# facebookresearch/EgoT2

Hardware: NVIDIA B200
Metric: translator fwd+bwd clips/sec (higher is better)
Workload: dtype bf16

## Files before the change

### egot2_b200/csrc/gemm_sm100.cu

```cuda
#include <stdio.h>
#include <stdlib.h>

#define EGOT2_FILE_ID 4
#include "ops.h"
#include "sm100.cuh"

namespace egot2 {

using namespace sm100;

namespace {

constexpr int BM = 128;
constexpr int BK = 64;
#ifndef EGOT2_GEMM_EPG
#define EGOT2_GEMM_EPG 1
#endif
constexpr int EPG = EGOT2_GEMM_EPG;
constexpr int NTHREADS = 64 + 128 * EPG;

struct EpiArgs {
  int M, N;
  void* C; int ldc; int c_rpg, c_gstride;
  const float* bias; int relu;
  const void* mask; int ldm; float mask_scale;
  float p_drop; uint64_t drop_key; int drop_bit_mode;
  const void* residual; int ldr;
  int accumulate; int atomic;
  long long split_stride;
  int tma_store;
  int k_grouped, kg, kdblocks;
  const float* ln_g; const float* ln_b; float ln_eps;
  void* ln_out; float* ln_stat; const float* ln_table; int ln_table_rows; int ln_row0;
  float ln_p_drop; uint64_t ln_drop_key;
  int trans_c;
  int tma_red;
  int trace_slot;
};

#ifdef EGOT2_GEMM_TRACE
__device__ long long g_gtrace[512][16];
#define GTR(k) do { if (blockIdx.x == 0 && blockIdx.z == 0 && e.trace_slot >= 0) g_gtrace[e.trace_slot][k] = clock64(); } while (0)
#else
#define GTR(k) do { } while (0)
#endif

__device__ __forceinline__ long long remap(int r, int rpg, int gstride) {
  return rpg > 0 ? (long long)(r / rpg) * gstride + (r % rpg) : (long long)r;
}


__device__ __forceinline__ void red_add_v4(float* p, float a, float b, float c, float d) {
  asm volatile("red.global.add.v4.f32 [%0], {%1, %2, %3, %4};" ::"l"(p), "f"(a), "f"(b), "f"(c), "f"(d) : "memory");
}

__device__ __forceinline__ bool aligned16(const void* p) { return (reinterpret_cast<uintptr_t>(p) & 15) == 0; }

__device__ __forceinline__ void load32(const float* p, float (&o)[32]) {
#pragma unroll
  for (int j = 0; j < 32; j += 4) {
    const float4 t = *reinterpret_cast<const float4*>(p + j);
    o[j] = t.x; o[j + 1] = t.y; o[j + 2] = t.z; o[j + 3] = t.w;
  }
}
__device__ __forceinline__ void load32(const bf16* p, float (&o)[32]) {
#pragma unroll
  for (int j = 0; j < 32; j += 8) {
    const uint4 t = *reinterpret_cast<const uint4*>(p + j);
    const uint32_t w[4] = {t.x, t.y, t.z, t.w};
#pragma unroll
    for (int k = 0; k < 4; ++k) {
      o[j + 2 * k] = __uint_as_float(w[k] << 16);
      o[j + 2 * k + 1] = __uint_as_float(w[k] & 0xffff0000u);
    }
  }
}
__device__ __forceinline__ void store32(float* p, const float (&v)[32]) {
#pragma unroll
  for (int j = 0; j < 32; j += 4) *reinterpret_cast<float4*>(p + j) = make_float4(v[j], v[j + 1], v[j + 2], v[j + 3]);
}
__device__ __forceinline__ void store32(bf16* p, const float (&v)[32]) {
#pragma unroll
  for (int j = 0; j < 32; j += 8) {
    uint4 o;
    __nv_bfloat162 p0 = __floats2bfloat162_rn(v[j], v[j + 1]), p1 = __floats2bfloat162_rn(v[j + 2], v[j + 3]);
    __nv_bfloat162 p2 = __floats2bfloat162_rn(v[j + 4], v[j + 5]), p3 = __floats2bfloat162_rn(v[j + 6], v[j + 7]);
    o.x = *reinterpret_cast<uint32_t*>(&p0); o.y = *reinterpret_cast<uint32_t*>(&p1);
    o.z = *reinterpret_cast<uint32_t*>(&p2); o.w = *reinterpret_cast<uint32_t*>(&p3);
    *reinterpret_cast<uint4*>(p + j) = o;
  }
}

template <int BN, typename TO> struct TileCfg {
  static constexpr uint32_t OUT_BYTES = (BN <= 128 && sizeof(TO) == 2) ? 128 * BN * 2 : 0;
  static constexpr int STAGES = BN == 128 ? (OUT_BYTES ? 2 : 3) : (BN == 64 ? (OUT_BYTES ? 3 : 4) : 4);
  static constexpr int MIN_CTAS = BN == 256 ? 1 : 2;
};
__device__ __forceinline__ void sts128(uint32_t dst, uint32_t a, uint32_t b, uint32_t c, uint32_t d) {
  asm volatile("st.shared.v4.b32 [%0], {%1, %2, %3, %4};" ::"r"(dst), "r"(a), "r"(b), "r"(c), "r"(d) : "memory");
}

__device__ __forceinline__ void named_bar_sync(int id, int n) { asm volatile("bar.sync %0, %1;" ::"r"(id), "r"(n) : "memory"); }

template <int BN, bool A_MN, bool B_MN, typename TO>
__global__ void __launch_bounds__(NTHREADS, TileCfg<BN, TO>::MIN_CTAS)
gemm_sm100_kernel(const __grid_constant__ CUtensorMap tma_a, const __grid_constant__ CUtensorMap tma_b,
                  const __grid_constant__ CUtensorMap tma_c, const EpiArgs e, const int k_blocks_total, const int k_blocks_per_split, const int tiles_n, const int num_tiles) {
  constexpr uint32_t A_BYTES = BM * BK * 2;
  constexpr uint32_t B_BYTES = BN * BK * 2;
  constexpr int STAGES = TileCfg<BN, TO>::STAGES;
  extern __shared__ uint8_t smem_raw[];
  const uint32_t smem_base = (smem_u32(smem_raw) + 1023u) & ~1023u;
  const uint32_t sA = smem_base;
  const uint32_t sB = sA + STAGES * A_BYTES;
  const uint32_t sOut = sB + STAGES * B_BYTES;
  const uint32_t bars = sOut + TileCfg<BN, TO>::OUT_BYTES;
  const uint32_t full0 = bars, empty0 = bars + 8 * STAGES, tmem_full = bars + 16 * STAGES, tmem_empty = tmem_full + 16;
  const uint32_t tmem_slot = tmem_empty + 16;
  const uint32_t bias_off = (tmem_slot + 8 + 15u) & ~15u;
  uint32_t* tmem_slot_ptr = reinterpret_cast<uint32_t*>(smem_raw + (tmem_slot - smem_u32(smem_raw)));

  const int warp = threadIdx.x >> 5, lane = threadIdx.x & 31;
  const int kb_begin = blockIdx.z * k_blocks_per_split;
  const int kb_end = min(k_blocks_total, kb_begin + k_blocks_per_split);
  const int nkb = kb_end - kb_begin;

  pdl_launch_dependents();
  if (threadIdx.x == 0) GTR(0);
  if (warp == 0 && lane == 0) {
    tma_prefetch_desc(&tma_a);
    tma_prefetch_desc(&tma_b);
    if (e.tma_store || e.tma_red) tma_prefetch_desc(&tma_c);
    for (int s = 0; s < STAGES; ++s) { mbar_init(full0 + 8 * s, 1); mbar_init(empty0 + 8 * s, 1); }
    for (int s = 0; s < 2; ++s) { mbar_init(tmem_full + 8 * s, 1); mbar_init(tmem_empty + 8 * s, 4 * EPG); }
    fence_barrier_init();
  }
  const bool one_tile = gridDim.z > 1;
  if (warp == 1) { if (one_tile) tmem_alloc<BN>(tmem_slot); else tmem_alloc<2 * BN>(tmem_slot); }
  if (threadIdx.x == 0) GTR(1);
  pdl_wait();
  if (threadIdx.x == 0) GTR(2);
  EGOT2_TL(EGOT2_FILE_ID);
  const unsigned long long egot2_ep = epoch_xor();
  float* sbias = reinterpret_cast<float*>(smem_raw + (bias_off - smem_u32(smem_raw)));
  tc_fence_before();
  __syncthreads();
  tc_fence_after();
  const uint32_t tmem_base = *tmem_slot_ptr;
  if (threadIdx.x == 0) GTR(3);

  if (warp == 0) {
    if (lane == 0) {
      int it = 0;
      for (int tile = blockIdx.x; tile < num_tiles; tile += gridDim.x) {
        const int m0 = (tile / tiles_n) * BM, n0 = (tile % tiles_n) * BN;
        for (int i = 0; i < nkb; ++i, ++it) {
          const int s = it % STAGES;
          const uint32_t ph = (it / STAGES) & 1;
          mbar_wait(empty0 + 8 * s, ph ^ 1);
          mbar_expect_tx(full0 + 8 * s, A_BYTES + B_BYTES);
          const int kb = kb_begin + i;
          const int k = kb * BK;
          if (A_MN && B_MN && e.k_grouped) {
            const int grp = (kb / e.kdblocks) * e.kg, d0 = (kb % e.kdblocks) * 64;
#pragma unroll
            for (int j = 0; j < BM / 64; ++j) tma_load_3d(sA + s * A_BYTES + j * 8192, &tma_a, full0 + 8 * s, m0 + 64 * j, d0, grp);
#pragma unroll
            for (int j = 0; j < BN / 64; ++j) tma_load_3d(sB + s * B_BYTES + j * 8192, &tma_b, full0 + 8 * s, n0 + 64 * j, d0, grp);
            continue;
          }
          if (!A_MN) {
            tma_load_2d(sA + s * A_BYTES, &tma_a, full0 + 8 * s, k, m0);
          } else {
#pragma unroll
            for (int j = 0; j < BM / 64; ++j) tma_load_2d(sA + s * A_BYTES + j * 8192, &tma_a, full0 + 8 * s, m0 + 64 * j, k);
          }
          if (!B_MN) {
            tma_load_2d(sB + s * B_BYTES, &tma_b, full0 + 8 * s, k, n0);
          } else {
#pragma unroll
            for (int j = 0; j < BN / 64; ++j) tma_load_2d(sB + s * B_BYTES + j * 8192, &tma_b, full0 + 8 * s, n0 + 64 * j, k);
          }
          if (tile == (int)blockIdx.x && (i == 0 || i == nkb - 1)) GTR(i == 0 ? 4 : 5);
        }
      }
    }
  } else if (warp == 1) {
    if (lane == 0) {
      constexpr uint32_t idesc = make_idesc_bf16(BM, BN, A_MN, B_MN);
      int it = 0, lt = 0;
      for (int tile = blockIdx.x; tile < num_tiles; tile += gridDim.x, ++lt) {
        const int buf = lt & 1;
        mbar_wait(tmem_empty + 8 * buf, ((lt >> 1) & 1) ^ 1);
        tc_fence_after();
        for (int i = 0; i < nkb; ++i, ++it) {
          const int s = it % STAGES;
          const uint32_t ph = (it / STAGES) & 1;
          mbar_wait(full0 + 8 * s, ph);
          if (lt == 0 && (i == 0 || i == nkb - 1)) GTR(i == 0 ? 6 : 7);
          tc_fence_after();
#pragma unroll
          for (int kk = 0; kk < BK / 16; ++kk) {
            const uint64_t ad = A_MN ? make_smem_desc_sw128(sA + s * A_BYTES + kk * 2048, 8192, 1024)
                                     : make_smem_desc_sw128(sA + s * A_BYTES + kk * 32, 16, 1024);
            const uint64_t bd = B_MN ? make_smem_desc_sw128(sB + s * B_BYTES + kk * 2048, 8192, 1024)
                                     : make_smem_desc_sw128(sB + s * B_BYTES + kk * 32, 16, 1024);
            umma_bf16(tmem_base + buf * BN, ad, bd, idesc, (i > 0 || kk > 0) ? 1u : 0u);
          }
          umma_commit(empty0 + 8 * s);
        }
        umma_commit(tmem_full + 8 * buf);
      }
    }
  } else {
    const int q = warp & 3;
    const int c_lo = ((warp - 2) >> 2) * (BN / EPG), c_hi = c_lo + BN / EPG;
    const float inv_keep = e.p_drop > 0.f ? 1.f / (1.f - e.p_drop) : 1.f;
    const bool first_split = blockIdx.z == 0;
    const float* bias = first_split ? e.bias : nullptr;
    const bool tma_red = sizeof(TO) == 4 && e.tma_red && gridDim.z > 1 && nkb > 0;
    int lt = 0;
    for (int tile = blockIdx.x; tile < num_tiles; tile += gridDim.x, ++lt) {
      const int buf = lt & 1;
      const int m0 = (tile / tiles_n) * BM, n0 = (tile % tiles_n) * BN;
      const int m = m0 + q * 32 + lane;
      float* sb = sbias + buf * BN;
      if (bias) {
        for (int i = threadIdx.x - 64; i < BN; i += NTHREADS - 64) sb[i] = n0 + i < e.N ? __ldg(bias + n0 + i) : 0.f;
        named_bar_sync(1, NTHREADS - 64);
      }
      const bool row_ok = (m < e.M) && nkb > 0;
      const long long crow = row_ok ? remap(m, e.c_rpg, e.c_gstride) : 0;
      TO* __restrict__ crow_ptr = (TO*)e.C + (long long)blockIdx.z * e.split_stride + crow * e.ldc;
      const TO* mask_row = e.mask ? (const TO*)e.mask + (long long)(row_ok ? m : 0) * e.ldm : nullptr;
      const TO* res_row = (e.residual && first_split) ? (const TO*)e.residual + (long long)(row_ok ? m : 0) * e.ldr : nullptr;
      const bool vec_ok = aligned16(crow_ptr) && aligned16(mask_row) && aligned16(res_row);
      const TO* aux_row = mask_row ? mask_row : res_row;
      float aux[32], aux_next[32];
      const bool aux_vec = row_ok && vec_ok && aux_row != nullptr;
      if (aux_vec && n0 + c_lo + 32 <= e.N) load32(aux_row + n0 + c_lo, aux_next);
      if (e.tma_store && lt > 0) {
        if (warp == 2 && lane == 0) tma_store_wait_read();
        named_bar_sync(3, NTHREADS - 64);
      }
      mbar_wait(tmem_full + 8 * buf, (lt >> 1) & 1);
      if (lt == 0 && threadIdx.x == 64) GTR(8);
      tc_fence_after();
      float ln_sum = 0.f, ln_sq = 0.f;
      if (tma_red) {
        const int rr = q * 32 + lane;
        uint32_t ra[32], rb[32];
        auto stage = [&](const uint32_t (&r)[32], int c0) {
          const uint32_t wbox = sA + (uint32_t)(c0 >> 5) * 16384u + (uint32_t)(q * 32) * 128u;
          if (e.trans_c) {
#pragma unroll
            for (int j = 0; j < 32; ++j)
              asm volatile("st.shared.b32 [%0], %1;" ::"r"(wbox + (uint32_t)j * 128u + (uint32_t)((((lane >> 2) ^ (j & 7)) << 4) | ((lane & 3) << 2))), "r"(r[j]) : "memory");
          } else {
            const uint32_t srow = wbox + (uint32_t)lane * 128u;
#pragma unroll
            for (int j = 0; j < 8; ++j) sts128(srow + (uint32_t)((j ^ (rr & 7)) << 4), r[4 * j], r[4 * j + 1], r[4 * j + 2], r[4 * j + 3]);
          }
          fence_proxy_async();
          __syncwarp();
          if (lane == 0 && n0 + c0 < e.N) {
            if (e.trans_c) tma_reduce_add_2d(&tma_c, wbox, m0 + q * 32, n0 + c0);
            else tma_reduce_add_2d(&tma_c, wbox, n0 + c0, m0 + q * 32);
          }
        };
        const uint32_t tcol = tmem_base + ((uint32_t)(q * 32) << 16) + (uint32_t)(buf * BN);
        tmem_ld_32x32(tcol + c_lo, ra);
#pragma unroll 1
        for (int c0 = c_lo; c0 < c_hi; c0 += 64) {
          tmem_ld_wait();
          if (c0 + 32 < c_hi) tmem_ld_32x32(tcol + c0 + 32, rb);
          stage(ra, c0);
          if (c0 + 32 < c_hi) {
            tmem_ld_wait();
            if (c0 + 64 < c_hi) tmem_ld_32x32(tcol + c0 + 64, ra);
            stage(rb, c0 + 32);
          }
        }
        tc_fence_before();
        __syncwarp();
        if (lane == 0) { mbar_arrive(tmem_empty + 8 * buf); tma_store_commit(); tma_store_wait_read(); }
        if (lt == 0 && threadIdx.x == 64) GTR(9);
        continue;
      }
#pragma unroll 1
      for (int c0 = c_lo; c0 < c_hi; c0 += 32) {
        uint32_t r[32];
        tmem_ld_32x32(tmem_base + ((uint32_t)(q * 32) << 16) + (uint32_t)(buf * BN + c0), r);
        const int nb = n0 + c0;
        const bool active = row_ok && nb < e.N;
        const bool fast = active && vec_ok && (nb + 32 <= e.N);
#pragma unroll
        for (int j = 0; j < 32; ++j) aux[j] = aux_next[j];
        if (aux_vec && c0 + 32 < c_hi && nb + 64 <= e.N) load32(aux_row + nb + 32, aux_next);
        tmem_ld_wait();
        if (c0 + 32 >= c_hi) {
          tc_fence_before();
          __syncwarp();
          if (lane == 0) mbar_arrive(tmem_empty + 8 * buf);
        }
        if (!active) continue;
        float v[32];
#pragma unroll
        for (int j = 0; j < 32; ++j) v[j] = __uint_as_float(r[j]);
        if (fast) {
          if (bias) {
#pragma unroll
            for (int j = 0; j < 32; j += 4) {
              const float4 b4 = *reinterpret_cast<const float4*>(sb + c0 + j);
              v[j] += b4.x; v[j + 1] += b4.y; v[j + 2] += b4.z; v[j + 3] += b4.w;
            }
          }
          if (e.relu) {
#pragma unroll
            for (int j = 0; j < 32; ++j) v[j] = fmaxf(v[j], 0.f);
          }
          if (mask_row) {
#pragma unroll
            for (int j = 0; j < 32; ++j) v[j] = aux[j] > 0.f ? v[j] * e.mask_scale : 0.f;
          }
          if (e.p_drop > 0.f) {
            const uint64_t idx0 = (uint64_t)m * e.N + nb;
            if (e.p_drop == 0.5f && (idx0 & 31) == 0) {
              const uint32_t kw = drop_word(e.drop_key ^ egot2_ep, idx0);
#pragma unroll
              for (int j = 0; j < 32; ++j) v[j] = (kw >> j) & 1u ? v[j] * inv_keep : 0.f;
            } else if (e.p_drop != 0.5f && (idx0 & 1) == 0) {
              float dm[32];
              drop_scale_n<32>(e.drop_key ^ egot2_ep, idx0, e.p_drop, inv_keep, dm);
#pragma unroll
              for (int j = 0; j < 32; ++j) v[j] *= dm[j];
            } else {
#pragma unroll
              for (int j = 0; j < 32; ++j) v[j] *= drop_scale(e.drop_key ^ egot2_ep, idx0 + j, e.p_drop, inv_keep);
            }
          }
          if (res_row) {
            if (mask_row) load32(res_row + nb, aux);
#pragma unroll
            for (int j = 0; j < 32; ++j) v[j] += aux[j];
          }
          if (e.accumulate) {
            if constexpr (sizeof(TO) == 4) {
              float* dst = (float*)crow_ptr + nb;
              if (e.atomic) {
#pragma unroll
                for (int j = 0; j < 32; j += 4) red_add_v4(dst + j, v[j], v[j + 1], v[j + 2], v[j + 3]);
              } else {
                float old[32];
                load32(dst, old);
#pragma unroll
                for (int j = 0; j < 32; ++j) v[j] += old[j];
                store32(dst, v);
              }
            }
          } else if (BN <= 128 && sizeof(TO) == 2 && (e.tma_store || e.ln_g)) {
            const int r = q * 32 + lane;
            const uint32_t srow = sOut + (uint32_t)(c0 >> 6) * 16384u + (uint32_t)r * 128u;
#pragma unroll
            for (int j = 0; j < 4; ++j) {
              uint32_t w[4];
#pragma unroll
              for (int k = 0; k < 4; ++k) {
                __nv_bfloat162 t = __floats2bfloat162_rn(v[8 * j + 2 * k], v[8 * j + 2 * k + 1]);
                w[k] = *reinterpret_cast<uint32_t*>(&t);
                if (e.ln_g) {
                  const float y0 = __uint_as_float(w[k] << 16), y1 = __uint_as_float(w[k] & 0xffff0000u);
                  ln_sum += y0 + y1;
                  ln_sq = fmaf(y0, y0, fmaf(y1, y1, ln_sq));
                }
              }
              sts128(srow + (uint32_t)(((((c0 & 63) >> 3) + j) ^ (r & 7)) << 4), w[0], w[1], w[2], w[3]);
            }
            if (!e.tma_store) store32(crow_ptr + nb, v);
          } else {
            store32(crow_ptr + nb, v);
          }
        } else {
#pragma unroll
          for (int j = 0; j < 32; ++j) {
            const int n = nb + j;
            if (n >= e.N) continue;
            float x = v[j];
            if (bias) x += sb[c0 + j];
            if (e.relu) x = fmaxf(x, 0.f);
            if (mask_row) x = to_f32(mask_row[n]) > 0.f ? x * e.mask_scale : 0.f;
            if (e.p_drop > 0.f) x *= drop_scale(e.drop_key ^ egot2_ep, (uint64_t)m * e.N + n, e.p_drop, inv_keep, e.drop_bit_mode != 0);
            if (res_row) x += to_f32(res_row[n]);
            if (e.accumulate) {
              if constexpr (sizeof(TO) == 4) {
                if (e.atomic) atomicAdd((float*)crow_ptr + n, x);
                else ((float*)crow_ptr)[n] += x;
              }
            } else {
              crow_ptr[n] = from_f32<TO>(x);
            }
          }
        }
      }
      if constexpr (BN == 128 && sizeof(TO) == 2) {
        if (e.ln_g && row_ok) {
          const float mean = ln_sum * (1.f / 128.f);
          const float rstd = rsqrtf(fmaxf(ln_sq * (1.f / 128.f) - mean * mean, 0.f) + e.ln_eps);
          const long long lrow = crow + e.ln_row0;
          if (e.ln_stat) { e.ln_stat[2 * lrow] = mean; e.ln_stat[2 * lrow + 1] = rstd; }
          bf16* orow = (bf16*)e.ln_out + crow * e.ldc;
          const float* trow = e.ln_table ? e.ln_table + (lrow % e.ln_table_rows) * 128 : nullptr;
          const float ln_keep = e.ln_p_drop > 0.f ? 1.f / (1.f - e.ln_p_drop) : 1.f;
          const int r = q * 32 + lane;
#pragma unroll 1
          for (int c0 = 0; c0 < 128; c0 += 32) {
            const uint32_t srow = sOut + (uint32_t)(c0 >> 6) * 16384u + (uint32_t)r * 128u;
#pragma unroll
            for (int j = 0; j < 4; ++j) {
              uint32_t w0, w1, w2, w3;
              asm volatile("ld.shared.v4.b32 {%0, %1, %2, %3}, [%4];" : "=r"(w0), "=r"(w1), "=r"(w2), "=r"(w3)
                           : "r"(srow + (uint32_t)(((((c0 & 63) >> 3) + j) ^ (r & 7)) << 4)));
              const uint32_t w[4] = {w0, w1, w2, w3};
              const int c = c0 + 8 * j;
              const float4 g0 = __ldg(reinterpret_cast<const float4*>(e.ln_g + c)), g1 = __ldg(reinterpret_cast<const float4*>(e.ln_g + c + 4));
              const float4 b0 = __ldg(reinterpret_cast<const float4*>(e.ln_b + c)), b1 = __ldg(reinterpret_cast<const float4*>(e.ln_b + c + 4));
              const float gg[8] = {g0.x, g0.y, g0.z, g0.w, g1.x, g1.y, g1.z, g1.w}, bb[8] = {b0.x, b0.y, b0.z, b0.w, b1.x, b1.y, b1.z, b1.w};
              float o[8];
#pragma unroll
              for (int k = 0; k < 4; ++k) {
                o[2 * k] = (__uint_as_float(w[k] << 16) - mean) * rstd * gg[2 * k] + bb[2 * k];
                o[2 * k + 1] = (__uint_as_float(w[k] & 0xffff0000u) - mean) * rstd * gg[2 * k + 1] + bb[2 * k + 1];
              }
              if (trow) {
                const float4 t0 = __ldg(reinterpret_cast<const float4*>(trow + c)), t1 = __ldg(reinterpret_cast<const float4*>(trow + c + 4));
                o[0] += t0.x; o[1] += t0.y; o[2] += t0.z; o[3] += t0.w; o[4] += t1.x; o[5] += t1.y; o[6] += t1.z; o[7] += t1.w;
              }
              if (e.ln_p_drop > 0.f) {
                { float dm[8]; drop_scale_n<8>(e.ln_drop_key ^ egot2_ep, (uint64_t)lrow * 128 + c, e.ln_p_drop, ln_keep, dm);
#pragma unroll
                  for (int k = 0; k < 8; ++k) o[k] *= dm[k]; }
              }
              uint4 pk;
              __nv_bfloat162 p0 = __floats2bfloat162_rn(o[0], o[1]), p1 = __floats2bfloat162_rn(o[2], o[3]);
              __nv_bfloat162 p2 = __floats2bfloat162_rn(o[4], o[5]), p3 = __floats2bfloat162_rn(o[6], o[7]);
              pk.x = *reinterpret_cast<uint32_t*>(&p0); pk.y = *reinterpret_cast<uint32_t*>(&p1);
              pk.z = *reinterpret_cast<uint32_t*>(&p2); pk.w = *reinterpret_cast<uint32_t*>(&p3);
              *reinterpret_cast<uint4*>(orow + c) = pk;
            }
          }
        }
      }
      if (lt == 0 && threadIdx.x == 64) GTR(9);
      if (BN <= 128 && e.tma_store) {
        fence_proxy_async();
        named_bar_sync(2, NTHREADS - 64);
        if (lt == 0 && threadIdx.x == 64) GTR(10);
        if (warp == 2 && lane == 0) {
#pragma unroll
          for (int h = 0; h < BN / 64; ++h) tma_store_2d(&tma_c, sOut + h * 16384, n0 + h * 64, m0);
          tma_store_commit();
        }
      }
    }
    if (e.tma_store && warp == 2 && lane == 0) tma_store_wait_all();
    if (threadIdx.x == 64) GTR(11);
  }
  tc_fence_before();
  __syncthreads();
  if (threadIdx.x == 0) GTR(12);
  if (warp == 1) {
    __syncwarp();
    if (one_tile) tmem_dealloc<BN>(tmem_base); else tmem_dealloc<2 * BN>(tmem_base);
    if (lane == 0) GTR(13);
  }
}

typedef CUresult (*EncodeTiledFn)(CUtensorMap*, CUtensorMapDataType, cuuint32_t, void*, const cuuint64_t*,
                                  const cuuint64_t*, const cuuint32_t*, const cuuint32_t*, CUtensorMapInterleave,
                                  CUtensorMapSwizzle, CUtensorMapL2promotion, CUtensorMapFloatOOBfill);

EncodeTiledFn encode_fn() {
  static EncodeTiledFn fn = nullptr;
  static bool tried = false;
  if (!tried) {
    tried = true;
    void* p = nullptr;
    cudaDriverEntryPointQueryResult qres;
    if (cudaGetDriverEntryPoint("cuTensorMapEncodeTiled", &p, cudaEnableDefault, &qres) == cudaSuccess &&
        qres == cudaDriverEntryPointSuccess)
      fn = (EncodeTiledFn)p;
  }
  return fn;
}

int make_map(CUtensorMap* map, const void* base, int inner, int rows, int ld, int box_inner, int box_rows) {
  EncodeTiledFn fn = encode_fn();
  EGOT2_CHECK(fn != nullptr, "cuTensorMapEncodeTiled not available from the driver");
  cuuint64_t dims[2] = {(cuuint64_t)inner, (cuuint64_t)rows};
  cuuint64_t strides[1] = {(cuuint64_t)ld * 2};
  cuuint32_t box[2] = {(cuuint32_t)box_inner, (cuuint32_t)box_rows};
  cuuint32_t estr[2] = {1, 1};
  CUresult r = fn(map, CU_TENSOR_MAP_DATA_TYPE_BFLOAT16, 2, const_cast<void*>(base), dims, strides, box, estr,
                  CU_TENSOR_MAP_INTERLEAVE_NONE, CU_TENSOR_MAP_SWIZZLE_128B, CU_TENSOR_MAP_L2_PROMOTION_L2_256B,
                  CU_TENSOR_MAP_FLOAT_OOB_FILL_NONE);
  EGOT2_CHECK(r == CUDA_SUCCESS, "cuTensorMapEncodeTiled failed (%d) inner=%d rows=%d ld=%d", (int)r, inner, rows, ld);
  return 0;
}

int make_map_f32(CUtensorMap* map, const void* base, int inner, int rows, int ld, int box_inner, int box_rows) {
  EncodeTiledFn fn = encode_fn();
  EGOT2_CHECK(fn != nullptr, "cuTensorMapEncodeTiled not available from the driver");
  cuuint64_t dims[2] = {(cuuint64_t)inner, (cuuint64_t)rows};
  cuuint64_t strides[1] = {(cuuint64_t)ld * 4};
  cuuint32_t box[2] = {(cuuint32_t)box_inner, (cuuint32_t)box_rows};
  cuuint32_t estr[2] = {1, 1};
  CUresult r = fn(map, CU_TENSOR_MAP_DATA_TYPE_FLOAT32, 2, const_cast<void*>(base), dims, strides, box, estr,
                  CU_TENSOR_MAP_INTERLEAVE_NONE, CU_TENSOR_MAP_SWIZZLE_128B, CU_TENSOR_MAP_L2_PROMOTION_L2_256B,
                  CU_TENSOR_MAP_FLOAT_OOB_FILL_NONE);
  EGOT2_CHECK(r == CUDA_SUCCESS, "cuTensorMapEncodeTiled(f32) failed (%d) inner=%d rows=%d ld=%d", (int)r, inner, rows, ld);
  return 0;
}

int make_map3(CUtensorMap* map, const void* base, int inner, int rpg, int groups, int ld, long long gstride_rows,
              int box_inner, int box_d, int box_g) {
  EncodeTiledFn fn = encode_fn();
  EGOT2_CHECK(fn != nullptr, "cuTensorMapEncodeTiled not available from the driver");
  cuuint64_t dims[3] = {(cuuint64_t)inner, (cuuint64_t)rpg, (cuuint64_t)groups};
  cuuint64_t strides[2] = {(cuuint64_t)ld * 2, (cuuint64_t)gstride_rows * ld * 2};
  cuuint32_t box[3] = {(cuuint32_t)box_inner, (cuuint32_t)box_d, (cuuint32_t)box_g};
  cuuint32_t estr[3] = {1, 1, 1};
  CUresult r = fn(map, CU_TENSOR_MAP_DATA_TYPE_BFLOAT16, 3, const_cast<void*>(base), dims, strides, box, estr,
                  CU_TENSOR_MAP_INTERLEAVE_NONE, CU_TENSOR_MAP_SWIZZLE_128B, CU_TENSOR_MAP_L2_PROMOTION_L2_256B,
                  CU_TENSOR_MAP_FLOAT_OOB_FILL_NONE);
  EGOT2_CHECK(r == CUDA_SUCCESS, "cuTensorMapEncodeTiled(3d) failed (%d) inner=%d rpg=%d groups=%d ld=%d", (int)r, inner,
              rpg, groups, ld);
  return 0;
}

struct KGroup { int on = 0, g = 1, dblocks = 1, kb_total = 0; };
#ifdef EGOT2_GEMM_TRACE
struct GTraceTag { char txt[96]; };
GTraceTag g_gtrace_tags[512];
int g_gtrace_n = 0;
#endif
static bool host_al16(const void* p) { return (reinterpret_cast<uintptr_t>(p) & 15) == 0; }

template <int BN, bool A_MN, bool B_MN, typename TO>
int launch(const GemmArgs& a, const CUtensorMap& ma, const CUtensorMap& mb, const KGroup& kg, cudaStream_t st) {
  constexpr int STAGES = TileCfg<BN, TO>::STAGES;
  constexpr size_t smem = 1024 + STAGES * (BM * BK * 2 + BN * BK * 2) + TileCfg<BN, TO>::OUT_BYTES + 16 * STAGES + 96 + 2 * BN * 4;
  static bool attr_set = false;
  auto kern = gemm_sm100_kernel<BN, A_MN, B_MN, TO>;
  if (!attr_set) {
    EGOT2_CUDA(cudaFuncSetAttribute(kern, cudaFuncAttributeMaxDynamicSharedMemorySize, (int)smem));
    attr_set = true;
  }
  EpiArgs e;
  e.M = a.M; e.N = a.N; e.C = a.C; e.ldc = a.ldc; e.c_rpg = a.c_rpg; e.c_gstride = a.c_gstride;
  e.bias = a.bias; e.relu = a.relu; e.mask = a.mask; e.ldm = a.ldm; e.mask_scale = a.mask_scale;
  e.p_drop = a.p_drop; e.drop_key = a.drop_key; e.drop_bit_mode = a.drop_bit_mode; e.residual = a.residual; e.ldr = a.ldr;
  e.accumulate = a.accumulate; e.atomic = a.split_k > 1;
  e.ln_g = a.ln_g; e.ln_b = a.ln_b; e.ln_eps = a.ln_eps; e.ln_out = a.ln_out; e.ln_stat = a.ln_stat; e.ln_table = a.ln_table;
  e.ln_table_rows = a.ln_table_rows > 0 ? a.ln_table_rows : 1; e.ln_row0 = a.ln_row0; e.ln_p_drop = a.ln_p_drop; e.ln_drop_key = a.ln_drop_key;
  e.k_grouped = kg.on; e.kg = kg.g; e.kdblocks = kg.dblocks;
  CUtensorMap mc = ma;
  e.tma_store = 0;
  if (BN <= 128 && sizeof(TO) == 2 && !a.accumulate && a.c_rpg == 0 && a.N % 32 == 0 && a.ldc % 8 == 0 && host_al16(a.C) &&
      (!a.mask || (host_al16(a.mask) && a.ldm % 8 == 0)) && (!a.residual || (host_al16(a.residual) && a.ldr % 8 == 0)) &&
      !(getenv("EGOT2_GEMM_TMASTORE") && getenv("EGOT2_GEMM_TMASTORE")[0] == '0')) {
    EGOT2_TRY(make_map(&mc, a.C, a.N, a.M, a.ldc, 64, 128));
    e.tma_store = 1;
  }
  const int kb_total = kg.on ? kg.kb_total : (a.K + BK - 1) / BK;
  int splits = a.split_k < 1 ? 1 : a.split_k;
  if (splits > kb_total) splits = kb_total;
  {
    const int nt = ((a.N + BN - 1) / BN) * ((a.M + BM - 1) / BM), slots = sm_count() * TileCfg<BN, TO>::MIN_CTAS;
    if (splits > 1 && nt * splits > slots) splits = slots / nt > 0 ? slots / nt : 1;
  }
  const int kb_per = (kb_total + splits - 1) / splits;
  splits = (kb_total + kb_per - 1) / kb_per;
  e.atomic = splits > 1 && a.split_stride == 0;
  e.split_stride = a.split_stride;
  static const bool tma_red_on = !(getenv("EGOT2_GEMM_TMARED") && getenv("EGOT2_GEMM_TMARED")[0] == '0');
  e.tma_red = 0;
  if (sizeof(TO) == 4 && tma_red_on && e.atomic && a.accumulate && !a.bias && !a.residual && !a.relu && !a.mask && a.p_drop <= 0.f &&
      a.c_rpg == 0 && a.N % 32 == 0 && a.ldc % 4 == 0 && host_al16(a.C) && (size_t)(BN / 32) * 16384 <= (size_t)STAGES * (BM * BK * 2 + BN * BK * 2)) {
    if (a.trans_c) EGOT2_TRY(make_map_f32(&mc, a.C, a.M, a.N, a.ldc, 32, 32));
    else EGOT2_TRY(make_map_f32(&mc, a.C, a.N, a.M, a.ldc, 32, 32));
    e.tma_red = 1;
  }
  e.trans_c = a.trans_c;
  if (a.trans_c && !e.tma_red) return -3;
  if (a.splits_out) *a.splits_out = splits;
  const int tiles_n = (a.N + BN - 1) / BN, num_tiles = tiles_n * ((a.M + BM - 1) / BM);
  int ctas = num_tiles;
  if (splits == 1) {
    const int slots = sm_count() * TileCfg<BN, TO>::MIN_CTAS;
    const int rounds = (num_tiles + slots - 1) / slots;
    ctas = (num_tiles + rounds - 1) / rounds;
  }
  dim3 grid(ctas, 1, splits);
  e.trace_slot = -1;
// ... 112 lines not shown
```

### egot2_b200/csrc/sm100.cuh

```cuda
#pragma once
#include <cuda.h>
#include <stdint.h>

namespace egot2 {
namespace sm100 {

__device__ __forceinline__ uint32_t smem_u32(const void* p) { return (uint32_t)__cvta_generic_to_shared(p); }

__device__ __forceinline__ void mbar_init(uint32_t bar, uint32_t count) {
  asm volatile("mbarrier.init.shared::cta.b64 [%0], %1;" ::"r"(bar), "r"(count) : "memory");
}
__device__ __forceinline__ void fence_barrier_init() {
  asm volatile("fence.mbarrier_init.release.cluster;" ::: "memory");
}
__device__ __forceinline__ void fence_proxy_async() { asm volatile("fence.proxy.async.shared::cta;" ::: "memory"); }
__device__ __forceinline__ void mbar_expect_tx(uint32_t bar, uint32_t bytes) {
  asm volatile("mbarrier.arrive.expect_tx.shared::cta.b64 _, [%0], %1;" ::"r"(bar), "r"(bytes) : "memory");
}
__device__ __forceinline__ void mbar_arrive(uint32_t bar) {
  asm volatile("mbarrier.arrive.shared::cta.b64 _, [%0];" ::"r"(bar) : "memory");
}
__device__ __forceinline__ bool mbar_try_wait(uint32_t bar, uint32_t parity) {
  uint32_t ok;
  asm volatile(
// ... 105 lines not shown
      "{\n\t.reg .pred p;\n\t"
      "setp.ne.b32 p, %4, 0;\n\t"
      "tcgen05.mma.cta_group::1.kind::f16 [%0], %1, %2, %3, p;\n\t}"
      ::"r"(d_tmem), "l"(adesc), "l"(bdesc), "r"(idesc), "r"(accumulate) : "memory");
}
__device__ __forceinline__ void umma_commit(uint32_t bar) {
  asm volatile("tcgen05.commit.cta_group::1.mbarrier::arrive::one.shared::cluster.b64 [%0];" ::"r"(bar) : "memory");
}

__device__ __forceinline__ void umma_commit_mc(uint32_t bar, uint16_t cta_mask) {
  asm volatile("tcgen05.commit.cta_group::1.mbarrier::arrive::one.shared::cluster.multicast::cluster.b64 [%0], %1;"
               ::"r"(bar), "h"(cta_mask) : "memory");
}

__device__ __forceinline__ void umma_bf16_cg2(uint32_t d_tmem, uint64_t adesc, uint64_t bdesc, uint32_t idesc, uint32_t accumulate) {
  asm volatile(
      "{\n\t.reg .pred p;\n\t"
      "setp.ne.b32 p, %4, 0;\n\t"
      "tcgen05.mma.cta_group::2.kind::f16 [%0], %1, %2, %3, p;\n\t}"
      ::"r"(d_tmem), "l"(adesc), "l"(bdesc), "r"(idesc), "r"(accumulate) : "memory");
}
__device__ __forceinline__ void umma_bf16_cg2_ts(uint32_t d_tmem, uint32_t a_tmem, uint64_t bdesc, uint32_t idesc, uint32_t accumulate) {
  asm volatile(
      "{\n\t.reg .pred p;\n\t"
      "setp.ne.b32 p, %4, 0;\n\t"
      "tcgen05.mma.cta_group::2.kind::f16 [%0], [%1], %2, %3, p;\n\t}"
      ::"r"(d_tmem), "r"(a_tmem), "l"(bdesc), "r"(idesc), "r"(accumulate) : "memory");
}
__device__ __forceinline__ void umma_commit_cg2(uint32_t bar, uint16_t cta_mask) {
  asm volatile("tcgen05.commit.cta_group::2.mbarrier::arrive::one.shared::cluster.multicast::cluster.b64 [%0], %1;"
               ::"r"(bar), "h"(cta_mask) : "memory");
}

__host__ __device__ constexpr uint32_t make_idesc_bf16(int M, int N, bool a_mn, bool b_mn) {
  return (1u << 4) | (1u << 7) | (1u << 10) | ((a_mn ? 1u : 0u) << 15) | ((b_mn ? 1u : 0u) << 16) |
         ((uint32_t)(N >> 3) << 17) | ((uint32_t)(M >> 4) << 24);
}
__device__ __forceinline__ uint64_t make_smem_desc_sw128(uint32_t saddr, uint32_t lbo_bytes, uint32_t sbo_bytes) {
  return (uint64_t)((saddr >> 4) & 0x3FFF) | ((uint64_t)((lbo_bytes >> 4) & 0x3FFF) << 16) |
         ((uint64_t)((sbo_bytes >> 4) & 0x3FFF) << 32) | (1ull << 46) | (2ull << 61);
}

__device__ __forceinline__ void tmem_ld_32x32(uint32_t taddr, uint32_t (&r)[32]) {
  asm volatile(
      "tcgen05.ld.sync.aligned.32x32b.x32.b32 "
      "{%0, %1, %2, %3, %4, %5, %6, %7, %8, %9, %10, %11, %12, %13, %14, %15, "
      "%16, %17, %18, %19, %20, %21, %22, %23, %24, %25, %26, %27, %28, %29, %30, %31}, [%32];"
      : "=r"(r[0]), "=r"(r[1]), "=r"(r[2]), "=r"(r[3]), "=r"(r[4]), "=r"(r[5]), "=r"(r[6]), "=r"(r[7]), "=r"(r[8]),
        "=r"(r[9]), "=r"(r[10]), "=r"(r[11]), "=r"(r[12]), "=r"(r[13]), "=r"(r[14]), "=r"(r[15]), "=r"(r[16]),
        "=r"(r[17]), "=r"(r[18]), "=r"(r[19]), "=r"(r[20]), "=r"(r[21]), "=r"(r[22]), "=r"(r[23]), "=r"(r[24]),
        "=r"(r[25]), "=r"(r[26]), "=r"(r[27]), "=r"(r[28]), "=r"(r[29]), "=r"(r[30]), "=r"(r[31])
      : "r"(taddr) : "memory");
}
__device__ __forceinline__ void tmem_ld_32x8(uint32_t taddr, uint32_t (&r)[8]) {
  asm volatile("tcgen05.ld.sync.aligned.32x32b.x8.b32 {%0, %1, %2, %3, %4, %5, %6, %7}, [%8];"
               : "=r"(r[0]), "=r"(r[1]), "=r"(r[2]), "=r"(r[3]), "=r"(r[4]), "=r"(r[5]), "=r"(r[6]), "=r"(r[7])
               : "r"(taddr) : "memory");
}
__device__ __forceinline__ void tmem_ld_wait() { asm volatile("tcgen05.wait::ld.sync.aligned;" ::: "memory"); }
__device__ __forceinline__ void tmem_st_32x32(uint32_t taddr, const uint32_t (&r)[32]) {
  asm volatile(
      "tcgen05.st.sync.aligned.32x32b.x32.b32 [%0], "
      "{%1, %2, %3, %4, %5, %6, %7, %8, %9, %10, %11, %12, %13, %14, %15, %16, "
      "%17, %18, %19, %20, %21, %22, %23, %24, %25, %26, %27, %28, %29, %30, %31, %32};"
      ::"r"(taddr), "r"(r[0]), "r"(r[1]), "r"(r[2]), "r"(r[3]), "r"(r[4]), "r"(r[5]), "r"(r[6]), "r"(r[7]), "r"(r[8]),
        "r"(r[9]), "r"(r[10]), "r"(r[11]), "r"(r[12]), "r"(r[13]), "r"(r[14]), "r"(r[15]), "r"(r[16]), "r"(r[17]),
        "r"(r[18]), "r"(r[19]), "r"(r[20]), "r"(r[21]), "r"(r[22]), "r"(r[23]), "r"(r[24]), "r"(r[25]), "r"(r[26]),
        "r"(r[27]), "r"(r[28]), "r"(r[29]), "r"(r[30]), "r"(r[31])
      : "memory");
}
__device__ __forceinline__ void tmem_st_wait() { asm volatile("tcgen05.wait::st.sync.aligned;" ::: "memory"); }

}
}
```

Measured before the change: 779,900.

## Double epilogue warps to 8 and split columns in halves with 16-wide TMEM loads

Fixes the GEMM epilogue at two warpgroups (256 threads), each handling half of the tile's columns, where the default before was one warpgroup. Epilogue chunks shrink from 32 to 16 columns using a new tcgen05.ld x16 helper. The fused LayerNorm epilogue now exchanges partial row sums through shared memory with a named barrier across both halves. The aim is to shorten the epilogue's critical path and cut register pressure, at the cost of more threads per CTA, extra shared memory and a barrier in the LN path.

```diff
diff --git a/egot2_b200/csrc/gemm_sm100.cu b/egot2_b200/csrc/gemm_sm100.cu
--- a/egot2_b200/csrc/gemm_sm100.cu
+++ b/egot2_b200/csrc/gemm_sm100.cu
@@ -13,11 +13,8 @@
 
 constexpr int BM = 128;
 constexpr int BK = 64;
-#ifndef EGOT2_GEMM_EPG
-#define EGOT2_GEMM_EPG 1
-#endif
-constexpr int EPG = EGOT2_GEMM_EPG;
-constexpr int NTHREADS = 64 + 128 * EPG;
+constexpr int NTHREADS = 64 + 256;
+constexpr int EPI_THREADS = NTHREADS - 64;
 
 struct EpiArgs {
   int M, N;
@@ -56,16 +53,16 @@
 
 __device__ __forceinline__ bool aligned16(const void* p) { return (reinterpret_cast<uintptr_t>(p) & 15) == 0; }
 
-__device__ __forceinline__ void load32(const float* p, float (&o)[32]) {
-#pragma unroll
-  for (int j = 0; j < 32; j += 4) {
+__device__ __forceinline__ void load16(const float* p, float (&o)[16]) {
+#pragma unroll
+  for (int j = 0; j < 16; j += 4) {
     const float4 t = *reinterpret_cast<const float4*>(p + j);
     o[j] = t.x; o[j + 1] = t.y; o[j + 2] = t.z; o[j + 3] = t.w;
   }
 }
-__device__ __forceinline__ void load32(const bf16* p, float (&o)[32]) {
-#pragma unroll
-  for (int j = 0; j < 32; j += 8) {
+__device__ __forceinline__ void load16(const bf16* p, float (&o)[16]) {
+#pragma unroll
+  for (int j = 0; j < 16; j += 8) {
     const uint4 t = *reinterpret_cast<const uint4*>(p + j);
     const uint32_t w[4] = {t.x, t.y, t.z, t.w};
 #pragma unroll
@@ -75,13 +72,13 @@
     }
   }
 }
-__device__ __forceinline__ void store32(float* p, const float (&v)[32]) {
-#pragma unroll
-  for (int j = 0; j < 32; j += 4) *reinterpret_cast<float4*>(p + j) = make_float4(v[j], v[j + 1], v[j + 2], v[j + 3]);
-}
-__device__ __forceinline__ void store32(bf16* p, const float (&v)[32]) {
-#pragma unroll
-  for (int j = 0; j < 32; j += 8) {
+__device__ __forceinline__ void store16(float* p, const float (&v)[16]) {
+#pragma unroll
+  for (int j = 0; j < 16; j += 4) *reinterpret_cast<float4*>(p + j) = make_float4(v[j], v[j + 1], v[j + 2], v[j + 3]);
+}
+__device__ __forceinline__ void store16(bf16* p, const float (&v)[16]) {
+#pragma unroll
+  for (int j = 0; j < 16; j += 8) {
     uint4 o;
     __nv_bfloat162 p0 = __floats2bfloat162_rn(v[j], v[j + 1]), p1 = __floats2bfloat162_rn(v[j + 2], v[j + 3]);
     __nv_bfloat162 p2 = __floats2bfloat162_rn(v[j + 4], v[j + 5]), p3 = __floats2bfloat162_rn(v[j + 6], v[j + 7]);
@@ -95,6 +92,7 @@
   static constexpr uint32_t OUT_BYTES = (BN <= 128 && sizeof(TO) == 2) ? 128 * BN * 2 : 0;
   static constexpr int STAGES = BN == 128 ? (OUT_BYTES ? 2 : 3) : (BN == 64 ? (OUT_BYTES ? 3 : 4) : 4);
   static constexpr int MIN_CTAS = BN == 256 ? 1 : 2;
+  static constexpr uint32_t LN_BYTES = (BN == 128 && sizeof(TO) == 2) ? 2 * 2 * 128 * 8 : 0;
 };
 __device__ __forceinline__ void sts128(uint32_t dst, uint32_t a, uint32_t b, uint32_t c, uint32_t d) {
   asm volatile("st.shared.v4.b32 [%0], {%1, %2, %3, %4};" ::"r"(dst), "r"(a), "r"(b), "r"(c), "r"(d) : "memory");
@@ -132,7 +130,7 @@
     tma_prefetch_desc(&tma_b);
     if (e.tma_store || e.tma_red) tma_prefetch_desc(&tma_c);
     for (int s = 0; s < STAGES; ++s) { mbar_init(full0 + 8 * s, 1); mbar_init(empty0 + 8 * s, 1); }
-    for (int s = 0; s < 2; ++s) { mbar_init(tmem_full + 8 * s, 1); mbar_init(tmem_empty + 8 * s, 4 * EPG); }
+    for (int s = 0; s < 2; ++s) { mbar_init(tmem_full + 8 * s, 1); mbar_init(tmem_empty + 8 * s, EPI_THREADS / 32); }
     fence_barrier_init();
   }
   const bool one_tile = gridDim.z > 1;
@@ -146,7 +144,6 @@
   tc_fence_before();
   __syncthreads();
   tc_fence_after();
-  const uint32_t tmem_base = *tmem_slot_ptr;
   if (threadIdx.x == 0) GTR(3);
 
   if (warp == 0) {
@@ -188,6 +185,7 @@
   } else if (warp == 1) {
     if (lane == 0) {
       constexpr uint32_t idesc = make_idesc_bf16(BM, BN, A_MN, B_MN);
+      const uint32_t tmem_base = *tmem_slot_ptr;
       int it = 0, lt = 0;
       for (int tile = blockIdx.x; tile < num_tiles; tile += gridDim.x, ++lt) {
         const int buf = lt & 1;
@@ -214,7 +212,8 @@
     }
   } else {
     const int q = warp & 3;
-    const int c_lo = ((warp - 2) >> 2) * (BN / EPG), c_hi = c_lo + BN / EPG;
+    const int half = (warp - 2) >> 2;
+    const int c_lo = half * (BN / 2), c_hi = c_lo + BN / 2;
     const float inv_keep = e.p_drop > 0.f ? 1.f / (1.f - e.p_drop) : 1.f;
     const bool first_split = blockIdx.z == 0;
     const float* bias = first_split ? e.bias : nullptr;
@@ -226,8 +225,8 @@
       const int m = m0 + q * 32 + lane;
       float* sb = sbias + buf * BN;
       if (bias) {
-        for (int i = threadIdx.x - 64; i < BN; i += NTHREADS - 64) sb[i] = n0 + i < e.N ? __ldg(bias + n0 + i) : 0.f;
-        named_bar_sync(1, NTHREADS - 64);
+        for (int i = threadIdx.x - 64; i < BN; i += EPI_THREADS) sb[i] = n0 + i < e.N ? __ldg(bias + n0 + i) : 0.f;
+        named_bar_sync(1, EPI_THREADS);
       }
       const bool row_ok = (m < e.M) && nkb > 0;
       const long long crow = row_ok ? remap(m, e.c_rpg, e.c_gstride) : 0;
@@ -236,49 +235,48 @@
       const TO* res_row = (e.residual && first_split) ? (const TO*)e.residual + (long long)(row_ok ? m : 0) * e.ldr : nullptr;
       const bool vec_ok = aligned16(crow_ptr) && aligned16(mask_row) && aligned16(res_row);
       const TO* aux_row = mask_row ? mask_row : res_row;
-      float aux[32], aux_next[32];
+      float aux[16], aux_next[16];
       const bool aux_vec = row_ok && vec_ok && aux_row != nullptr;
-      if (aux_vec && n0 + c_lo + 32 <= e.N) load32(aux_row + n0 + c_lo, aux_next);
+      if (aux_vec && n0 + c_lo + 16 <= e.N) load16(aux_row + n0 + c_lo, aux_next);
       if (e.tma_store && lt > 0) {
         if (warp == 2 && lane == 0) tma_store_wait_read();
-        named_bar_sync(3, NTHREADS - 64);
+        named_bar_sync(3, EPI_THREADS);
       }
       mbar_wait(tmem_full + 8 * buf, (lt >> 1) & 1);
       if (lt == 0 && threadIdx.x == 64) GTR(8);
       tc_fence_after();
+      const uint32_t tacc = *tmem_slot_ptr + ((uint32_t)(q * 32) << 16) + (uint32_t)(buf * BN);
       float ln_sum = 0.f, ln_sq = 0.f;
       if (tma_red) {
         const int rr = q * 32 + lane;
-        uint32_t ra[32], rb[32];
-        auto stage = [&](const uint32_t (&r)[32], int c0) {
+        uint32_t ra[16], rb[16];
+        auto stage = [&](const uint32_t (&r)[16], int c0, int h) {
           const uint32_t wbox = sA + (uint32_t)(c0 >> 5) * 16384u + (uint32_t)(q * 32) * 128u;
           if (e.trans_c) {
 #pragma unroll
-            for (int j = 0; j < 32; ++j)
-              asm volatile("st.shared.b32 [%0], %1;" ::"r"(wbox + (uint32_t)j * 128u + (uint32_t)((((lane >> 2) ^ (j & 7)) << 4) | ((lane & 3) << 2))), "r"(r[j]) : "memory");
+            for (int j = 0; j < 16; ++j)
+              asm volatile("st.shared.b32 [%0], %1;" ::"r"(wbox + (uint32_t)(16 * h + j) * 128u + (uint32_t)((((lane >> 2) ^ (j & 7)) << 4) | ((lane & 3) << 2))), "r"(r[j]) : "memory");
           } else {
             const uint32_t srow = wbox + (uint32_t)lane * 128u;
 #pragma unroll
-            for (int j = 0; j < 8; ++j) sts128(srow + (uint32_t)((j ^ (rr & 7)) << 4), r[4 * j], r[4 * j + 1], r[4 * j + 2], r[4 * j + 3]);
-          }
+            for (int j = 0; j < 4; ++j) sts128(srow + (uint32_t)(((4 * h + j) ^ (rr & 7)) << 4), r[4 * j], r[4 * j + 1], r[4 * j + 2], r[4 * j + 3]);
+          }
+        };
+        tmem_ld_32x16(tacc + c_lo, ra);
+#pragma unroll 1
+        for (int c0 = c_lo; c0 < c_hi; c0 += 32) {
+          tmem_ld_wait();
+          tmem_ld_32x16(tacc + c0 + 16, rb);
+          stage(ra, c0, 0);
+          tmem_ld_wait();
+          if (c0 + 32 < c_hi) tmem_ld_32x16(tacc + c0 + 32, ra);
+          stage(rb, c0, 1);
           fence_proxy_async();
           __syncwarp();
           if (lane == 0 && n0 + c0 < e.N) {
+            const uint32_t wbox = sA + (uint32_t)(c0 >> 5) * 16384u + (uint32_t)(q * 32) * 128u;
             if (e.trans_c) tma_reduce_add_2d(&tma_c, wbox, m0 + q * 32, n0 + c0);
             else tma_reduce_add_2d(&tma_c, wbox, n0 + c0, m0 + q * 32);
-          }
-        };
-        const uint32_t tcol = tmem_base + ((uint32_t)(q * 32) << 16) + (uint32_t)(buf * BN);
-        tmem_ld_32x32(tcol + c_lo, ra);
-#pragma unroll 1
-        for (int c0 = c_lo; c0 < c_hi; c0 += 64) {
-          tmem_ld_wait();
-          if (c0 + 32 < c_hi) tmem_ld_32x32(tcol + c0 + 32, rb);
-          stage(ra, c0);
-          if (c0 + 32 < c_hi) {
-            tmem_ld_wait();
-            if (c0 + 64 < c_hi) tmem_ld_32x32(tcol + c0 + 64, ra);
-            stage(rb, c0 + 32);
           }
         }
         tc_fence_before();
@@ -288,81 +286,81 @@
         continue;
       }
 #pragma unroll 1
-      for (int c0 = c_lo; c0 < c_hi; c0 += 32) {
-        uint32_t r[32];
-        tmem_ld_32x32(tmem_base + ((uint32_t)(q * 32) << 16) + (uint32_t)(buf * BN + c0), r);
+      for (int c0 = c_lo; c0 < c_hi; c0 += 16) {
+        uint32_t r[16];
+        tmem_ld_32x16(tacc + (uint32_t)c0, r);
         const int nb = n0 + c0;
         const bool active = row_ok && nb < e.N;
-        const bool fast = active && vec_ok && (nb + 32 <= e.N);
-#pragma unroll
-        for (int j = 0; j < 32; ++j) aux[j] = aux_next[j];
-        if (aux_vec && c0 + 32 < c_hi && nb + 64 <= e.N) load32(aux_row + nb + 32, aux_next);
+        const bool fast = active && vec_ok && (nb + 16 <= e.N);
+#pragma unroll
+        for (int j = 0; j < 16; ++j) aux[j] = aux_next[j];
+        if (aux_vec && c0 + 16 < c_hi && nb + 32 <= e.N) load16(aux_row + nb + 16, aux_next);
         tmem_ld_wait();
-        if (c0 + 32 >= c_hi) {
+        if (c0 + 16 >= c_hi) {
           tc_fence_before();
           __syncwarp();
           if (lane == 0) mbar_arrive(tmem_empty + 8 * buf);
         }
         if (!active) continue;
-        float v[32];
-#pragma unroll
-        for (int j = 0; j < 32; ++j) v[j] = __uint_as_float(r[j]);
+        float v[16];
+#pragma unroll
+        for (int j = 0; j < 16; ++j) v[j] = __uint_as_float(r[j]);
         if (fast) {
           if (bias) {
 #pragma unroll
-            for (int j = 0; j < 32; j += 4) {
+            for (int j = 0; j < 16; j += 4) {
               const float4 b4 = *reinterpret_cast<const float4*>(sb + c0 + j);
               v[j] += b4.x; v[j + 1] += b4.y; v[j + 2] += b4.z; v[j + 3] += b4.w;
             }
           }
           if (e.relu) {
 #pragma unroll
-            for (int j = 0; j < 32; ++j) v[j] = fmaxf(v[j], 0.f);
+            for (int j = 0; j < 16; ++j) v[j] = fmaxf(v[j], 0.f);
           }
           if (mask_row) {
 #pragma unroll
-            for (int j = 0; j < 32; ++j) v[j] = aux[j] > 0.f ? v[j] * e.mask_scale : 0.f;
+            for (int j = 0; j < 16; ++j) v[j] = aux[j] > 0.f ? v[j] * e.mask_scale : 0.f;
           }
           if (e.p_drop > 0.f) {
             const uint64_t idx0 = (uint64_t)m * e.N + nb;
-            if (e.p_drop == 0.5f && (idx0 & 31) == 0) {
+            if (e.p_drop == 0.5f && (idx0 & 15) == 0) {
               const uint32_t kw = drop_word(e.drop_key ^ egot2_ep, idx0);
 #pragma unroll
-              for (int j = 0; j < 32; ++j) v[j] = (kw >> j) & 1u ? v[j] * inv_keep : 0.f;
+              for (int j = 0; j < 16; ++j) v[j] = (kw >> j) & 1u ? v[j] * inv_keep : 0.f;
             } else if (e.p_drop != 0.5f && (idx0 & 1) == 0) {
-              float dm[32];
-              drop_scale_n<32>(e.drop_key ^ egot2_ep, idx0, e.p_drop, inv_keep, dm);
-#pragma unroll
-              for (int j = 0; j < 32; ++j) v[j] *= dm[j];
+              float dm[16];
+              drop_scale_n<16>(e.drop_key ^ egot2_ep, idx0, e.p_drop, inv_keep, dm);
+#pragma unroll
+              for (int j = 0; j < 16; ++j) v[j] *= dm[j];
             } else {
 #pragma unroll
-              for (int j = 0; j < 32; ++j) v[j] *= drop_scale(e.drop_key ^ egot2_ep, idx0 + j, e.p_drop, inv_keep);
+              for (int j = 0; j < 16; ++j) v[j] *= drop_scale(e.drop_key ^ egot2_ep, idx0 + j, e.p_drop, inv_keep);
             }
           }
           if (res_row) {
-            if (mask_row) load32(res_row + nb, aux);
-#pragma unroll
-            for (int j = 0; j < 32; ++j) v[j] += aux[j];
+            if (mask_row) load16(res_row + nb, aux);
+#pragma unroll
+            for (int j = 0; j < 16; ++j) v[j] += aux[j];
           }
           if (e.accumulate) {
             if constexpr (sizeof(TO) == 4) {
               float* dst = (float*)crow_ptr + nb;
               if (e.atomic) {
 #pragma unroll
-                for (int j = 0; j < 32; j += 4) red_add_v4(dst + j, v[j], v[j + 1], v[j + 2], v[j + 3]);
+                for (int j = 0; j < 16; j += 4) red_add_v4(dst + j, v[j], v[j + 1], v[j + 2], v[j + 3]);
               } else {
-                float old[32];
-                load32(dst, old);
-#pragma unroll
-                for (int j = 0; j < 32; ++j) v[j] += old[j];
-                store32(dst, v);
+                float old[16];
+                load16(dst, old);
+#pragma unroll
+                for (int j = 0; j < 16; ++j) v[j] += old[j];
+                store16(dst, v);
               }
             }
           } else if (BN <= 128 && sizeof(TO) == 2 && (e.tma_store || e.ln_g)) {
             const int r = q * 32 + lane;
             const uint32_t srow = sOut + (uint32_t)(c0 >> 6) * 16384u + (uint32_t)r * 128u;
 #pragma unroll
-            for (int j = 0; j < 4; ++j) {
+            for (int j = 0; j < 2; ++j) {
               uint32_t w[4];
 #pragma unroll
               for (int k = 0; k < 4; ++k) {
@@ -376,13 +374,13 @@
               }
               sts128(srow + (uint32_t)(((((c0 & 63) >> 3) + j) ^ (r & 7)) << 4), w[0], w[1], w[2], w[3]);
             }
-            if (!e.tma_store) store32(crow_ptr + nb, v);
+            if (!e.tma_store) store16(crow_ptr + nb, v);
           } else {
-            store32(crow_ptr + nb, v);
+            store16(crow_ptr + nb, v);
           }
         } else {
 #pragma unroll
-          for (int j = 0; j < 32; ++j) {
+          for (int j = 0; j < 16; ++j) {
             const int n = nb + j;
             if (n >= e.N) continue;
             float x = v[j];
@@ -403,49 +401,57 @@
         }
       }
       if constexpr (BN == 128 && sizeof(TO) == 2) {
-        if (e.ln_g && row_ok) {
-          const float mean = ln_sum * (1.f / 128.f);
-          const float rstd = rsqrtf(fmaxf(ln_sq * (1.f / 128.f) - mean * mean, 0.f) + e.ln_eps);
-          const long long lrow = crow + e.ln_row0;
-          if (e.ln_stat) { e.ln_stat[2 * lrow] = mean; e.ln_stat[2 * lrow + 1] = rstd; }
-          bf16* orow = (bf16*)e.ln_out + crow * e.ldc;
-          const float* trow = e.ln_table ? e.ln_table + (lrow % e.ln_table_rows) * 128 : nullptr;
-          const float ln_keep = e.ln_p_drop > 0.f ? 1.f / (1.f - e.ln_p_drop) : 1.f;
+        if (e.ln_g) {
           const int r = q * 32 + lane;
+          float2* sln = reinterpret_cast<float2*>(sbias + 2 * BN) + buf * 256;
+          sln[half * 128 + r] = make_float2(ln_sum, ln_sq);
+          named_bar_sync(4, EPI_THREADS);
+          const float2 o = sln[(half ^ 1) * 128 + r];
+          ln_sum += o.x;
+          ln_sq += o.y;
+          if (row_ok) {
+            const float mean = ln_sum * (1.f / 128.f);
+            const float rstd = rsqrtf(fmaxf(ln_sq * (1.f / 128.f) - mean * mean, 0.f) + e.ln_eps);
+            const long long lrow = crow + e.ln_row0;
+            if (e.ln_stat && half == 0) { e.ln_stat[2 * lrow] = mean; e.ln_stat[2 * lrow + 1] = rstd; }
+            bf16* orow = (bf16*)e.ln_out + crow * e.ldc;
+            const float* trow = e.ln_table ? e.ln_table + (lrow % e.ln_table_rows) * 128 : nullptr;
+            const float ln_keep = e.ln_p_drop > 0.f ? 1.f / (1.f - e.ln_p_drop) : 1.f;
 #pragma unroll 1
-          for (int c0 = 0; c0 < 128; c0 += 32) {
-            const uint32_t srow = sOut + (uint32_t)(c0 >> 6) * 16384u + (uint32_t)r * 128u;
-#pragma unroll
-            for (int j = 0; j < 4; ++j) {
-              uint32_t w0, w1, w2, w3;
-              asm volatile("ld.shared.v4.b32 {%0, %1, %2, %3}, [%4];" : "=r"(w0), "=r"(w1), "=r"(w2), "=r"(w3)
-                           : "r"(srow + (uint32_t)(((((c0 & 63) >> 3) + j) ^ (r & 7)) << 4)));
-              const uint32_t w[4] = {w0, w1, w2, w3};
-              const int c = c0 + 8 * j;
-              const float4 g0 = __ldg(reinterpret_cast<const float4*>(e.ln_g + c)), g1 = __ldg(reinterpret_cast<const float4*>(e.ln_g + c + 4));
-              const float4 b0 = __ldg(reinterpret_cast<const float4*>(e.ln_b + c)), b1 = __ldg(reinterpret_cast<const float4*>(e.ln_b + c + 4));
-              const float gg[8] = {g0.x, g0.y, g0.z, g0.w, g1.x, g1.y, g1.z, g1.w}, bb[8] = {b0.x, b0.y, b0.z, b0.w, b1.x, b1.y, b1.z, b1.w};
-              float o[8];
-#pragma unroll
-              for (int k = 0; k < 4; ++k) {
-                o[2 * k] = (__uint_as_float(w[k] << 16) - mean) * rstd * gg[2 * k] + bb[2 * k];
-                o[2 * k + 1] = (__uint_as_float(w[k] & 0xffff0000u) - mean) * rstd * gg[2 * k + 1] + bb[2 * k + 1];
+            for (int c0 = c_lo; c0 < c_hi; c0 += 32) {
+              const uint32_t srow = sOut + (uint32_t)(c0 >> 6) * 16384u + (uint32_t)r * 128u;
+#pragma unroll
+              for (int j = 0; j < 4; ++j) {
+                uint32_t w0, w1, w2, w3;
+                asm volatile("ld.shared.v4.b32 {%0, %1, %2, %3}, [%4];" : "=r"(w0), "=r"(w1), "=r"(w2), "=r"(w3)
+                             : "r"(srow + (uint32_t)(((((c0 & 63) >> 3) + j) ^ (r & 7)) << 4)));
+                const uint32_t w[4] = {w0, w1, w2, w3};
+                const int c = c0 + 8 * j;
+                const float4 g0 = __ldg(reinterpret_cast<const float4*>(e.ln_g + c)), g1 = __ldg(reinterpret_cast<const float4*>(e.ln_g + c + 4));
+                const float4 b0 = __ldg(reinterpret_cast<const float4*>(e.ln_b + c)), b1 = __ldg(reinterpret_cast<const float4*>(e.ln_b + c + 4));
+                const float gg[8] = {g0.x, g0.y, g0.z, g0.w, g1.x, g1.y, g1.z, g1.w}, bb[8] = {b0.x, b0.y, b0.z, b0.w, b1.x, b1.y, b1.z, b1.w};
+                float o[8];
+#pragma unroll
+                for (int k = 0; k < 4; ++k) {
+                  o[2 * k] = (__uint_as_float(w[k] << 16) - mean) * rstd * gg[2 * k] + bb[2 * k];
+                  o[2 * k + 1] = (__uint_as_float(w[k] & 0xffff0000u) - mean) * rstd * gg[2 * k + 1] + bb[2 * k + 1];
+                }
+                if (trow) {
+                  const float4 t0 = __ldg(reinterpret_cast<const float4*>(trow + c)), t1 = __ldg(reinterpret_cast<const float4*>(trow + c + 4));
+                  o[0] += t0.x; o[1] += t0.y; o[2] += t0.z; o[3] += t0.w; o[4] += t1.x; o[5] += t1.y; o[6] += t1.z; o[7] += t1.w;
+                }
+                if (e.ln_p_drop > 0.f) {
+                  { float dm[8]; drop_scale_n<8>(e.ln_drop_key ^ egot2_ep, (uint64_t)lrow * 128 + c, e.ln_p_drop, ln_keep, dm);
+#pragma unroll
+                    for (int k = 0; k < 8; ++k) o[k] *= dm[k]; }
+                }
+                uint4 pk;
+                __nv_bfloat162 p0 = __floats2bfloat162_rn(o[0], o[1]), p1 = __floats2bfloat162_rn(o[2], o[3]);
+                __nv_bfloat162 p2 = __floats2bfloat162_rn(o[4], o[5]), p3 = __floats2bfloat162_rn(o[6], o[7]);
+                pk.x = *reinterpret_cast<uint32_t*>(&p0); pk.y = *reinterpret_cast<uint32_t*>(&p1);
+                pk.z = *reinterpret_cast<uint32_t*>(&p2); pk.w = *reinterpret_cast<uint32_t*>(&p3);
+                *reinterpret_cast<uint4*>(orow + c) = pk;
               }
-              if (trow) {
-                const float4 t0 = __ldg(reinterpret_cast<const float4*>(trow + c)), t1 = __ldg(reinterpret_cast<const float4*>(trow + c + 4));
-                o[0] += t0.x; o[1] += t0.y; o[2] += t0.z; o[3] += t0.w; o[4] += t1.x; o[5] += t1.y; o[6] += t1.z; o[7] += t1.w;
-              }
-              if (e.ln_p_drop > 0.f) {
-                { float dm[8]; drop_scale_n<8>(e.ln_drop_key ^ egot2_ep, (uint64_t)lrow * 128 + c, e.ln_p_drop, ln_keep, dm);
-#pragma unroll
-                  for (int k = 0; k < 8; ++k) o[k] *= dm[k]; }
-              }
-              uint4 pk;
-              __nv_bfloat162 p0 = __floats2bfloat162_rn(o[0], o[1]), p1 = __floats2bfloat162_rn(o[2], o[3]);
-              __nv_bfloat162 p2 = __floats2bfloat162_rn(o[4], o[5]), p3 = __floats2bfloat162_rn(o[6], o[7]);
-              pk.x = *reinterpret_cast<uint32_t*>(&p0); pk.y = *reinterpret_cast<uint32_t*>(&p1);
-              pk.z = *reinterpret_cast<uint32_t*>(&p2); pk.w = *reinterpret_cast<uint32_t*>(&p3);
-              *reinterpret_cast<uint4*>(orow + c) = pk;
             }
           }
         }
@@ -453,7 +459,7 @@
       if (lt == 0 && threadIdx.x == 64) GTR(9);
       if (BN <= 128 && e.tma_store) {
         fence_proxy_async();
-        named_bar_sync(2, NTHREADS - 64);
+        named_bar_sync(2, EPI_THREADS);
         if (lt == 0 && threadIdx.x == 64) GTR(10);
         if (warp == 2 && lane == 0) {
 #pragma unroll
@@ -470,6 +476,7 @@
   if (threadIdx.x == 0) GTR(12);
   if (warp == 1) {
     __syncwarp();
+    const uint32_t tmem_base = *tmem_slot_ptr;
     if (one_tile) tmem_dealloc<BN>(tmem_base); else tmem_dealloc<2 * BN>(tmem_base);
     if (lane == 0) GTR(13);
   }
@@ -548,7 +555,8 @@
 template <int BN, bool A_MN, bool B_MN, typename TO>
 int launch(const GemmArgs& a, const CUtensorMap& ma, const CUtensorMap& mb, const KGroup& kg, cudaStream_t st) {
   constexpr int STAGES = TileCfg<BN, TO>::STAGES;
-  constexpr size_t smem = 1024 + STAGES * (BM * BK * 2 + BN * BK * 2) + TileCfg<BN, TO>::OUT_BYTES + 16 * STAGES + 96 + 2 * BN * 4;
+  constexpr size_t smem = 1024 + STAGES * (BM * BK * 2 + BN * BK * 2) + TileCfg<BN, TO>::OUT_BYTES + 16 * STAGES + 96 + 2 * BN * 4 +
+                          TileCfg<BN, TO>::LN_BYTES;
   static bool attr_set = false;
   auto kern = gemm_sm100_kernel<BN, A_MN, B_MN, TO>;
   if (!attr_set) {
diff --git a/egot2_b200/csrc/sm100.cuh b/egot2_b200/csrc/sm100.cuh
--- a/egot2_b200/csrc/sm100.cuh
+++ b/egot2_b200/csrc/sm100.cuh
@@ -181,6 +181,14 @@
         "=r"(r[25]), "=r"(r[26]), "=r"(r[27]), "=r"(r[28]), "=r"(r[29]), "=r"(r[30]), "=r"(r[31])
       : "r"(taddr) : "memory");
 }
+__device__ __forceinline__ void tmem_ld_32x16(uint32_t taddr, uint32_t (&r)[16]) {
+  asm volatile(
+      "tcgen05.ld.sync.aligned.32x32b.x16.b32 "
+      "{%0, %1, %2, %3, %4, %5, %6, %7, %8, %9, %10, %11, %12, %13, %14, %15}, [%16];"
+      : "=r"(r[0]), "=r"(r[1]), "=r"(r[2]), "=r"(r[3]), "=r"(r[4]), "=r"(r[5]), "=r"(r[6]), "=r"(r[7]), "=r"(r[8]),
+        "=r"(r[9]), "=r"(r[10]), "=r"(r[11]), "=r"(r[12]), "=r"(r[13]), "=r"(r[14]), "=r"(r[15])
+      : "r"(taddr) : "memory");
+}
 __device__ __forceinline__ void tmem_ld_32x8(uint32_t taddr, uint32_t (&r)[8]) {
   asm volatile("tcgen05.ld.sync.aligned.32x32b.x8.b32 {%0, %1, %2, %3, %4, %5, %6, %7}, [%8];"
                : "=r"(r[0]), "=r"(r[1]), "=r"(r[2]), "=r"(r[3]), "=r"(r[4]), "=r"(r[5]), "=r"(r[6]), "=r"(r[7])
```

Measured after the change: 791,800 (median of 6 runs). +1.5%, better.
